# ethz-asl/object_keypoints

Measured on AMD Instinct MI355X. Metric: frames/sec keypoint inference (511x511 -> heatmaps+3D), higher is better.
Workload: dtype bf16; 1 GPU; BASELINE configs[2]: batch=64/GPU synthetic 511x511 frames, bf16 activations+weights, fp32 accumulate, CornerNet-Squeeze K=3 (valve) random-init procedural weights; fp32 NCHW frames -> stem -> hourglass+heads; peak-NMS -> depth lifting -> object grouping on injected bump scenes (SURVEY 8(d), 1-2 objects/frame); frames_per_gpu=64, global_batch=64, parallelism=frame-dp1, resident_frame_batches=4

## Files before the change

object_keypoints_amd/csrc/okp_fire2.hip:

```cpp
#include <cstdio>
#include <cstring>

#include <cstdlib>

#include "okp_internal.h"

#ifdef OKP_F2_ABL_NOSTORE
#define F2_STORE_(v, rs, off) do { if ((off) == 0x7ffffff0u) __builtin_amdgcn_raw_buffer_store_b128(v, rs, (int)(off), 0, 0); } while (0)
#else
#define F2_STORE_(v, rs, off) __builtin_amdgcn_raw_buffer_store_b128(v, rs, (int)(off), 0, 0)
#endif
#define F2_STORE(v, rs, off) do { \
    if constexpr (G) { if ((uint32_t)(off) < kInvalid) range_h = okp_range_max_h8(range_h, v); } \
    F2_STORE_(v, rs, off); } while (0)


namespace {

constexpr uint32_t kInvalid = 0x80000000u;
typedef __attribute__((address_space(3))) void* lds_ptr_t;
typedef float f32x2 __attribute__((ext_vector_type(2)));

constexpr int SP = 128;
constexpr int PBI = 6;
// ... 50 lines not shown
    case 5: asm volatile("s_waitcnt vmcnt(5)" ::: "memory"); break;
    case 6: asm volatile("s_waitcnt vmcnt(6)" ::: "memory"); break;
    case 7: asm volatile("s_waitcnt vmcnt(7)" ::: "memory"); break;
    default: asm volatile("s_waitcnt vmcnt(8)" ::: "memory"); break;
  }
}

#ifdef OKP_FIRE_STAMPS
#define F2_STAMP_ANY(i) do { if (lane == 0 && blockIdx.x < 16) { uint64_t t_; asm volatile("s_memtime %0\n s_waitcnt lgkmcnt(0)" : "=s"(t_) :: "memory"); p.dbg[(blockIdx.x * 8 + w) * 8 + (i)] = (uint32_t)t_; } } while (0)
#define F2_STAMP(i) do { if (second && lane == 0 && blockIdx.x < 16) { uint64_t t_; asm volatile("s_memtime %0\n s_waitcnt lgkmcnt(0)" : "=s"(t_) :: "memory"); p.dbg[(blockIdx.x * 8 + w) * 8 + (i)] = (uint32_t)t_; } } while (0)
#else
#define F2_STAMP(i) do {} while (0)
#define F2_STAMP_ANY(i) do {} while (0)
#endif

template <typename T, int CIN, int MID, int STR, bool DWM = false, bool G = false>
__global__ __launch_bounds__(MID * 2, MID == 128 ? 2 : 1) void okp_fire2_kernel(const OkpFire2Params p) {
  static_assert(STR == 1 || STR == 2, "stride of both branches");
  static_assert(!G || std::is_same<T, _Float16>::value, "the 16-bit storage guard is an fp16 instantiation");
  constexpr bool DWM2 = DWM && STR == 2;
  constexpr int D2H = 3, D2W = 8, D2SW = 2 * (D2W - 1) + 3, D2SH = 2 * (D2H - 1) + 3, D2B = 2;
  static_assert(D2SH * D2SW <= SP && D2B * 16 >= D2H * D2W + 8, "stride-2 matrix-pipe tile");
  constexpr int DIH = kDwmIH;
  constexpr int DSW = 18;
  constexpr int NSB = !DWM ? SP / 16 : STR == 1 ? ((DIH + 2) * DSW + 15) / 16 : (D2SH * D2SW + 15) / 16;
  constexpr int NW = MID / 32;
  constexpr int NT = 64 * NW;
  constexpr int HALF = MID;
  constexpr int KS1 = CIN / 32;
  constexpr int KS2 = MID / 32;
#ifdef OKP_F2_RESIDENT_W1
  constexpr bool RES = CIN <= 256;
  constexpr int DWB = 1;
#else
  constexpr bool RES = false;
#ifdef OKP_F2_RESIDENT_WA
  constexpr int DWB = (CIN == 256 && MID == 128) ? OKP_F2_RESIDENT_WA : 1;
#else
  constexpr int DWB = (CIN == 256 && MID == 128) ? 4 : 1;
#endif
// ... 94 lines not shown
    const int row = 16 * (w + NW * i) + (lane >> 2);
    d_sy[i] = fastdiv(row, p.div_sw);
    d_sx[i] = row - d_sy[i] * p.SW;
    if (row >= p.SH * p.SW) d_sy[i] = 1 << 20;
    d_chunk[i] = (uint32_t)(((lane & 3) - 2 * (row >> 2)) & 3) * 16u;
  }
  const int m_sy = tid < p.SH * p.SW ? fastdiv(tid, p.div_sw) : (1 << 20);
  const int m_sx = tid - fastdiv(tid, p.div_sw) * p.SW;

  auto tile_origin = [&](int slot, int& n, int& y0, int& x0) {
    const int xq = p.n_tiles >> 3, xr = p.n_tiles & 7, xcd = slot & 7;
    const int tile = (xcd < xr ? xcd * (xq + 1) : xr * (xq + 1) + (xcd - xr) * xq) + (slot >> 3);
    n = fastdiv(tile, p.div_tiles_frame);
    const int trem = tile - n * p.tiles_y * p.tiles_x;
    const int ty = fastdiv(trem, p.div_tiles_x);
    y0 = ty * p.IH;
    x0 = (trem - ty * p.tiles_x) * p.IW;
  };
  uint32_t d_off[NDM];
  auto tile_setup = [&](int tile) {
    int n, y0, x0;
    tile_origin(tile, n, y0, x0);
#pragma unroll
    for (int i = 0; i < NDM; ++i) {
      const int y = STR * y0 - 1 + d_sy[i], x = STR * x0 - 1 + d_sx[i];
      const bool ok = y >= 0 && y < p.H && x >= 0 && x < p.W;
      d_off[i] = ok ? (uint32_t)(((long)n * p.H + y) * p.W + x) * (uint32_t)(p.x_ps * 2) + d_chunk[i] : kInvalid;
    }
    if (tid < SP) {
      const int y = STR * y0 - 1 + m_sy, x = STR * x0 - 1 + m_sx;
      const unsigned long long m = __ballot(y >= 0 && y < p.H && x >= 0 && x < p.W);
      if (lane == 0) {
        uint32_t* mk = reinterpret_cast<uint32_t*>(smem + OFF_MASK);
        mk[2 * w] = (uint32_t)m;
        mk[2 * w + 1] = (uint32_t)(m >> 32);
      }
    }
  };
#ifdef OKP_F2_ABL_NOX
  bool abl_started = false;
#endif
  auto issue_x = [&](int ks, int stage) {
#ifdef OKP_F2_ABL_NOX
    if (abl_started) return;
#endif
#pragma unroll
    for (int i = 0; i < NDM; ++i)
      if (UNI || i < nd)
        __builtin_amdgcn_raw_ptr_buffer_load_lds(rs_x, (lds_ptr_t)(smem + OFF_X + stage * XST + (w + NW * i) * 1024), 16,
                                                 (int)(d_off[i] == kInvalid ? kInvalid : d_off[i] + (uint32_t)ks * 64u), 0, 0, 0);
  };

  int tile = blockIdx.x;
  if (tile >= p.n_tiles) return;
  F2_STAMP_ANY(5);
  tile_setup(tile);
  first_weights(w1f);
#pragma unroll
  for (int ks = 0; ks < NST - 1; ++ks) issue_x(ks, ks);
  {
    static_assert(10 * HALF == 5 * NT, "depth-wise constants per thread");
    float cv[5];
#pragma unroll
    for (int k = 0; k < 5; ++k) {
      const int i = tid + k * NT;
      cv[k] = *(i < 9 * HALF ? p.wd + i : p.bd + (i - 9 * HALF));
    }
#pragma unroll
    for (int k = 0; k < 5; ++k) {
      const int i = tid + k * NT;
      if constexpr (DWM) {
        const uint32_t wq = (i & 1) ? okp_pack2<T>(0.f, cv[k]) : okp_pack2<T>(cv[k], 0.f);
        reinterpret_cast<uint32_t*>(smem + OFF_WD)[i] = i < 9 * HALF ? wq : __builtin_bit_cast(uint32_t, cv[k]);
      } else {
        reinterpret_cast<float*>(smem + OFF_WD)[i] = cv[k];
      }
    }
  }
  if (tid < 16 * PBI) {
    const int iy = fastdiv(tid, p.div_iw), ix = tid - iy * p.IW;
    reinterpret_cast<uint32_t*>(smem + OFF_TAB)[tid] = tid < p.IP ? (uint32_t)(iy * p.W + ix) * (uint32_t)(p.x_ps * 2) : kInvalid;
    reinterpret_cast<uint32_t*>(smem + OFF_TAB)[96 + tid] = tid < p.IP ? (uint32_t)(iy * p.Wo + ix) * (uint32_t)(p.out_ps * 2) : kInvalid;
  }

  __syncthreads();
  F2_STAMP_ANY(6);

  uint32_t range_h = 0u;
  for (; tile < p.n_tiles; tile += gridDim.x) {
    int n, y0, x0;
    tile_origin(tile, n, y0, x0);
#ifdef OKP_FIRE_STAMPS
    const bool second = tile == (int)(blockIdx.x + gridDim.x);
#endif
    F2_STAMP(0);
    int qt = q, tidt = tid;
    asm volatile("" : "+v"(qt), "+v"(tidt));
#ifdef OKP_F2_NO_REMAP
    const int dw_cg = tidt % CG, dw_slot = tidt / CG;
#else
    const int dw_l = tidt & 31;
    const int dw_cg = CG == 16 ? ((dw_l & 3) | ((dw_l >> 1) & 12)) : tidt % CG;
    const int dw_slot = CG == 16 ? 4 * (tidt >> 6) + 2 * ((tidt >> 5) & 1) + (((dw_l >> 2) ^ (dw_l >> 3) ^ (dw_l >> 4)) & 1) : tidt / CG;
#endif
    auto load_col_residuals = [&](int ix, u32x4 (&rr)[MAXIH], uint32_t (&oo)[MAXIH]) {
      const int cg = dw_cg;
      const int ox = x0 + ix;
      const uint32_t pix = (uint32_t)(((long)n * p.Ho + y0) * p.Wo + ox);
// ... 9 lines not shown
            const int row = (iy + 1) * p.SW + (ix < p.IW ? ix : 0) + 1;
            rr[iy] = *reinterpret_cast<const u32x4*>(smem + OFF_X + ((KS1 / 2 + (cg >> 2)) % NST) * XST + row * 64 + (((cg & 3) + 2 * (row >> 2)) & 3) * 16);
          } else {
            rr[iy] = __builtin_amdgcn_raw_buffer_load_b128(rs_x, (int)(ok ? xo : kInvalid), 0, 0);
          }
        }
        xo += (uint32_t)(p.W * p.x_ps * 2);
        oof += (uint32_t)(p.Wo * p.out_ps * 2);
      }
    };
    uint32_t o_off[PBI];
    u32x4 r_raw[PBI];
    u32x4 rr[MAXIH];
    uint32_t oo[MAXIH];

    f32x4 acc[NSB][2];
#pragma unroll
    for (int pb = 0; pb < NSB; ++pb) {
      acc[pb][0] = b1v0;
      acc[pb][1] = b1v1;
    }
    if constexpr (PIPE) {
      u32x4 a[2][NSB];
#pragma unroll
      for (int ks = 0; ks <= KS1; ++ks) {
        if (ks < KS1) {
          if (ks == 0) wait_vm(0);
          else if (ks >= 3) wait_vm(2 + (ks + 1 < KS1 ? nd + 2 : 0) + (ks + 2 < KS1 ? nd : 0));
          asm volatile("s_waitcnt lgkmcnt(0)" ::: "memory");
          __builtin_amdgcn_s_barrier();
          if (ks + 2 < KS1) load_w1(ks + 2, w1f[(ks + 2) % NWS]);
          if (ks + NST - 1 < KS1) issue_x(ks + NST - 1, (ks + NST - 1) % NST);
          const char* st = smem + OFF_X + (ks % NST) * XST + xfrag_off;
#pragma unroll
          for (int pb = 0; pb < NSB; ++pb) a[ks & 1][pb] = *reinterpret_cast<const u32x4*>(st + pb * 1024);
          __builtin_amdgcn_sched_barrier(0);
        }
        if (ks > 0) {
#pragma unroll
          for (int pb = 0; pb < NSB; ++pb)
#pragma unroll
            for (int b = 0; b < 2; ++b)
              acc[pb][b] = H16<T>::mfma16(w1f[(ks - 1) % NWS][b], a[(ks - 1) & 1][pb], acc[pb][b]);
          __builtin_amdgcn_sched_barrier(0);
        }
      }
    } else
#pragma unroll
    for (int ks = 0; ks < KS1; ++ks) {
      if (ks == 0) wait_vm(0);
      else if constexpr (WRING) {
        auto nw = [](int j) { return j >= 1 && j - 1 + DW < KS1 ? 2 : 0; };
        auto nx = [](int j) { return j >= 0 && j + NST - 1 < KS1 ? 1 : 0; };
        wait_vm((DW >= 4 ? nw(ks - 2) : 0) + nw(ks - 1) + (nx(ks - 2) + nx(ks - 1)) * nd);
      } else if (ks >= (RES ? NST - 1 : 2))
        wait_vm((ks + 1 < KS1 ? nd + (RES ? 0 : 2) : 0) + (ks + 2 < KS1 ? nd : 0));
      asm volatile("s_waitcnt lgkmcnt(0)" ::: "memory");
      __builtin_amdgcn_s_barrier();
      if constexpr (WRING) { if (ks >= 1 && ks - 1 + DW < KS1) issue_w(ks - 1 + DW); }
      else if constexpr (!RES) { if (ks + 2 < KS1) load_w1(ks + 2, w1f[(ks + 2) % 3]); }
      if (ks + NST - 1 < KS1) issue_x(ks + NST - 1, (ks + NST - 1) % NST);
      const char* st = smem + OFF_X + (ks % NST) * XST + xfrag_off;
      u32x4 a[NSB], wr[2] = {};
      if constexpr (WRING) {
#pragma unroll
        for (int b = 0; b < 2; ++b) wr[b] = *reinterpret_cast<const u32x4*>(smem + OFF_W1 + ((ks % DW) * NW + w) * 2048 + b * 1024 + lane * 16);
      }
#pragma unroll
      for (int pb = 0; pb < NSB; ++pb) a[pb] = *reinterpret_cast<const u32x4*>(st + pb * 1024);
#ifdef OKP_F2_PIN_READS
      __builtin_amdgcn_sched_barrier(0);
#endif
#pragma unroll
      for (int pb = 0; pb < NSB; ++pb)
#pragma unroll
        for (int b = 0; b < 2; ++b)
          acc[pb][b] = H16<T>::mfma16(WRING ? wr[b] : w1f[RES ? ks : ks % 3][b], a[pb], acc[pb][b]);
    }
    F2_STAMP(1);
#ifdef OKP_F2_ABL_NOX
    abl_started = true;
#endif
    if constexpr (!RESWA) {
#pragma unroll
      for (int b = 0; b < 2; ++b)
#pragma unroll
        for (int ks = 0; ks < KS2; ++ks) {
#ifdef OKP_F2_ABL_NOWEIGHTS
          if (b + ks != 0) { waf[b][ks] = u32x4{0x3c003c00u, 0u, 0u, 0u}; continue; }
#endif
          waf[b][ks] = wa_lane[(size_t)(b * KS2 + ks) * 64];
        }
    }
    {
      const uint32_t* mk = reinterpret_cast<const uint32_t*>(smem + OFF_MASK);
      int l16t = l16;
      asm volatile("" : "+v"(l16t));
      uint32_t mq[4];
#pragma unroll
      for (int i = 0; i < 4; ++i) mq[i] = mk[i] >> l16t;
#pragma unroll
      for (int pb = 0; pb < NSB; ++pb) {
        const bool ok = (mq[pb >> 1] >> (16 * (pb & 1))) & 1u;
        u32x4 v;
#pragma unroll
        for (int b = 0; b < 2; ++b) {
          const uint32_t p0 = okp_pack2<T>(acc[pb][b][0], acc[pb][b][1]), p1 = okp_pack2<T>(acc[pb][b][2], acc[pb][b][3]);
          v[2 * b] = ok ? p0 : 0u;
          v[2 * b + 1] = ok ? p1 : 0u;
        }
        if constexpr (G) range_h = okp_range_max_h8(range_h, v);
        *reinterpret_cast<u32x4*>(smem + s_dst + pb * 16 * (MID * 2)) = v;
      }
    }
    __syncthreads();
    F2_STAMP(2);
    uint32_t dwm_o[DIH];
    uint32_t d2_o[D2B];
    if constexpr (DWM2) {
      int l16t = l16;
      asm volatile("" : "+v"(l16t));
      const int liy = l16t >> 3, lix = l16t & 7;
      const uint32_t pix0 = (uint32_t)(((long)n * p.Ho + y0) * p.Wo + x0);
      const uint32_t lane_o = (uint32_t)(liy * p.Wo + lix) * (uint32_t)(p.out_ps * 2) + (uint32_t)chq * 2u;
      const bool col_ok = lix < p.IW && x0 + lix < p.Wo;
      f32x4 ac2[D2B][2];
#pragma unroll
      for (int pb = 0; pb < D2B; ++pb) {
        const int iy = 2 * pb + liy;
        const bool ok = col_ok && iy < p.IH && y0 + iy < p.Ho;
        d2_o[pb] = ok ? lane_o + (pix0 + (uint32_t)(2 * pb * p.Wo)) * (uint32_t)(p.out_ps * 2) : kInvalid;
// ... 18 lines not shown
#pragma unroll
      for (int pb = 0; pb < D2B; ++pb) {
        const u32x4 v = relu_add_pack8<T>(ac2[pb][0], ac2[pb][1], u32x4{0u, 0u, 0u, 0u});
        F2_STORE(v, rs_o, d2_o[pb]);
      }
    } else if constexpr (DWM) {
      int l16t = l16;
      asm volatile("" : "+v"(l16t));
      const uint32_t pix0 = (uint32_t)(((long)n * p.Ho + y0) * p.Wo + x0);
      const uint32_t lane_x = (uint32_t)l16t * (uint32_t)(p.x_ps * 2) + (uint32_t)chq * 2u, lane_o = (uint32_t)l16t * (uint32_t)(p.out_ps * 2) + (uint32_t)chq * 2u;
      u32x4 rsk[DIH];
      const uint32_t rowx = (uint32_t)(p.W * p.x_ps * 2), rowo = (uint32_t)(p.Wo * p.out_ps * 2), noskip = p.skip ? 0u : kInvalid;
      uint32_t sx = pix0 * (uint32_t)(p.x_ps * 2), so = pix0 * (uint32_t)(p.out_ps * 2);
#pragma unroll
      for (int iy = 0; iy < DIH; ++iy) {
        const uint32_t bad = (iy < p.IH && y0 + iy < p.Ho) ? 0u : kInvalid;
        dwm_o[iy] = lane_o + (so | bad);
        rsk[iy] = __builtin_amdgcn_raw_buffer_load_b128(rs_x, (int)(lane_x + (sx | bad | noskip)), 0, 0);
        sx += rowx;
        so += rowo;
      }
      f32x4 ac2[DIH][2];
#pragma unroll
      for (int iy = 0; iy < DIH; ++iy) {
        ac2[iy][0] = bav0;
        ac2[iy][1] = bav1;
      }
      const uint32_t s_lane = (uint32_t)OFF_S + (uint32_t)(DSW + 1 + l16t) * (uint32_t)(MID * 2);
#pragma unroll
      for (int ks = 0; ks < KS2; ++ks) {
        u32x4 a[DIH];
#pragma unroll
        for (int iy = 0; iy < DIH; ++iy) {
          const uint32_t key = (uint32_t)(l16t + (iy + 1) * DSW + 1) & (uint32_t)SWM;
          a[iy] = *reinterpret_cast<const u32x4*>(smem + s_lane + (uint32_t)(iy * DSW * MID * 2) + (((uint32_t)(4 * ks + qt) ^ key) << 4));
        }
#pragma unroll
        for (int iy = 0; iy < DIH; ++iy)
#pragma unroll
          for (int b = 0; b < 2; ++b)
            ac2[iy][b] = H16<T>::mfma16(waf[b][ks], a[iy], ac2[iy][b]);
      }
#pragma unroll
      for (int iy = 0; iy < DIH; ++iy) {
        const u32x4 v = relu_add_pack8<T>(ac2[iy][0], ac2[iy][1], rsk[iy]);
        F2_STORE(v, rs_o, dwm_o[iy]);
      }
    } else {
      const bool full = y0 + p.IH <= p.Ho && x0 + p.IW <= p.Wo;
      const uint32_t pix0 = (uint32_t)(((long)n * p.Ho + y0) * p.Wo + x0);
// ... 38 lines not shown
      for (int pb = 0; pb < PBI; ++pb) {
        if (16 * pb < p.IP) {
          const u32x4 v = relu_add_pack8<T>(ac2[pb][0], ac2[pb][1], r_raw[pb]);
          F2_STORE(v, rs_o, o_off[pb]);
        }
      }
    }
    asm volatile("" ::: "memory");
    F2_STAMP(3);

    if constexpr (DWM2) {
      int l16t = l16;
      asm volatile("" : "+v"(l16t));
      const int liy = l16t >> 3, lix = l16t & 7;
      {
        const int next = tile + gridDim.x;
        if (next < p.n_tiles) {
          tile_setup(next);
          first_weights(w1f);
#pragma unroll
          for (int ks = 0; ks < NST - 1; ++ks) issue_x(ks, ks);
        }
      }
      const float* const bl = reinterpret_cast<const float*>(smem + OFF_WD) + 9 * HALF + chq;
      const f32x4 bdv0 = *reinterpret_cast<const f32x4*>(bl), bdv1 = *reinterpret_cast<const f32x4*>(bl + 4);
      f32x4 acd[D2B][2];
#pragma unroll
      for (int pb = 0; pb < D2B; ++pb) { acd[pb][0] = bdv0; acd[pb][1] = bdv1; }
      const uint32_t am = (qt == (l16t >> 2)) ? 0xffffffffu : 0u;
      const uint32_t m_lo = (l16t & 2) ? 0u : am, m_hi = (l16t & 2) ? am : 0u;
      const uint32_t wt_lane = (uint32_t)OFF_WD + (uint32_t)(chq + (l16t & 3)) * 4u;
      const uint32_t cx = (uint32_t)(4 * w) + (uint32_t)qt;
      const uint32_t sp_lane = (uint32_t)(2 * liy * D2SW + 2 * lix);
      u32x4 a0 = {0u, 0u, 0u, 0u}, a1 = {0u, 0u, 0u, 0u};
#pragma unroll
      for (int tap = 0; tap < 9; ++tap) {
        const int dy = tap / 3, dx = tap % 3;
// ... 17 lines not shown
      for (int pb = 0; pb < D2B; ++pb) {
        const u32x4 o = relu_add_pack8<T>(acd[pb][0], acd[pb][1], u32x4{0u, 0u, 0u, 0u});
        F2_STORE(o, rs_o, d2_o[pb] == kInvalid ? kInvalid : d2_o[pb] + (uint32_t)(HALF * 2));
      }
    } else if constexpr (DWM) {
      int l16t = l16;
      asm volatile("" : "+v"(l16t));
      u32x4 rr2[DIH];
      uint32_t oo2[DIH];
#pragma unroll
      for (int iy = 0; iy < DIH; ++iy) {
        oo2[iy] = dwm_o[iy] + (uint32_t)(HALF * 2);
        rr2[iy] = u32x4{0u, 0u, 0u, 0u};
        if (p.skip) {
          if constexpr (RING_SKIP) {
            const uint32_t row = (uint32_t)((iy + 1) * DSW + 1) + (uint32_t)l16t;
            rr2[iy] = *reinterpret_cast<const u32x4*>(smem + OFF_X + ((KS1 / 2 + w) % NST) * XST + row * 64u + (((uint32_t)qt + 2u * (row >> 2)) & 3u) * 16u);
          } else {
            const bool ok = iy < p.IH && y0 + iy < p.Ho;
            const uint32_t pix0 = (uint32_t)(((long)n * p.Ho + y0) * p.Wo + x0);
            const uint32_t sx = ok ? (pix0 + (uint32_t)(iy * p.W)) * (uint32_t)(p.x_ps * 2) : kInvalid;
            rr2[iy] = __builtin_amdgcn_raw_buffer_load_b128(rs_x, (int)((uint32_t)l16t * (uint32_t)(p.x_ps * 2) + (uint32_t)(HALF + chq) * 2u + sx), 0, 0);
          }
        }
      }
      if constexpr (RING_SKIP) {
        if (p.skip) { asm volatile("s_waitcnt lgkmcnt(0)" ::: "memory"); __syncthreads(); }
      }
      {
        const int next = tile + gridDim.x;
        if (next < p.n_tiles) {
          tile_setup(next);
          first_weights(w1f);
#pragma unroll
          for (int ks = 0; ks < NST - 1; ++ks) issue_x(ks, ks);
        }
      }
      const float* const bl = reinterpret_cast<const float*>(smem + OFF_WD) + 9 * HALF + chq;
      const f32x4 bdv0 = *reinterpret_cast<const f32x4*>(bl), bdv1 = *reinterpret_cast<const f32x4*>(bl + 4);
      f32x4 acd[DIH][2];
#pragma unroll
      for (int iy = 0; iy < DIH; ++iy) { acd[iy][0] = bdv0; acd[iy][1] = bdv1; }
      const uint32_t am = (qt == (l16t >> 2)) ? 0xffffffffu : 0u;
      const uint32_t m_lo = (l16t & 2) ? 0u : am, m_hi = (l16t & 2) ? am : 0u;
      const uint32_t wt_lane = (uint32_t)OFF_WD + (uint32_t)(chq + (l16t & 3)) * 4u;
      const uint32_t cx = (uint32_t)(4 * w) + (uint32_t)qt;
#ifndef OKP_F2_ABL_NODW
      u32x4 a0[3], a1[3];
#pragma unroll
      for (int dy = 0; dy < 3; ++dy) { a0[dy] = u32x4{0u, 0u, 0u, 0u}; a1[dy] = u32x4{0u, 0u, 0u, 0u}; }
#pragma unroll
      for (int dx = 0; dx < 3; ++dx) {
#pragma unroll
        for (int dy = 0; dy < 3; ++dy) {
          const uint32_t v0 = *reinterpret_cast<const uint32_t*>(smem + wt_lane + ((dy * 3 + dx) * HALF) * 4);
          const uint32_t v1 = *reinterpret_cast<const uint32_t*>(smem + wt_lane + ((dy * 3 + dx) * HALF + 4) * 4);
          a0[dy][0] = v0 & m_lo; a0[dy][1] = v0 & m_hi;
          a1[dy][2] = v1 & m_lo; a1[dy][3] = v1 & m_hi;
        }
        u32x4 bf[DIH + 2];
#pragma unroll
        for (int r = 0; r < DIH + 2; ++r) {
          const uint32_t sp = (uint32_t)(r * DSW + dx) + (uint32_t)l16t;
          bf[r] = *reinterpret_cast<const u32x4*>(smem + OFF_S + sp * (MID * 2) + ((cx ^ (sp & SWM)) << 4));
        }
#pragma unroll
        for (int r = 0; r < DIH + 2; ++r) {
#pragma unroll
          for (int dy = 0; dy < 3; ++dy) {
            const int iy = r - dy;
            if (iy >= 0 && iy < DIH) {
              acd[iy][0] = H16<T>::mfma16(a0[dy], bf[r], acd[iy][0]);
              acd[iy][1] = H16<T>::mfma16(a1[dy], bf[r], acd[iy][1]);
            }
          }
        }
      }
#endif
// ... 8 lines not shown
      const float* const wl = reinterpret_cast<const float*>(smem + OFF_WD) + cg * 8;
      float breg[8];
      {
        const f32x4 u0 = *reinterpret_cast<const f32x4*>(wl + 9 * HALF), u1 = *reinterpret_cast<const f32x4*>(wl + 9 * HALF + 4);
#pragma unroll
        for (int e = 0; e < 4; ++e) { breg[e] = u0[e]; breg[4 + e] = u1[e]; }
      }
      bool prefetched = false;
      for (int ix = dw_slot; ix < ((p.IW + 15) & ~15); ix += 16) {
        load_col_residuals(ix, rr, oo);
        if (RING_SKIP ? ix + 16 >= ((p.IW + 15) & ~15) : !prefetched) {
          prefetched = true;
          if constexpr (RING_SKIP) {
            if (p.skip) { asm volatile("s_waitcnt lgkmcnt(0)" ::: "memory"); __syncthreads(); }
          }
          const int next = tile + gridDim.x;
          if (next < p.n_tiles) {
            tile_setup(next);
            first_weights(w1f);
#pragma unroll
            for (int ks = 0; ks < NST - 1; ++ks) issue_x(ks, ks);
          }
        }
        const int ixc = ix < p.IW ? ix : 0;
        f32x2 v[MAXIH][4];
#pragma unroll
        for (int iy = 0; iy < MAXIH; ++iy)
#pragma unroll
          for (int e = 0; e < 4; ++e) v[iy][e] = f32x2{breg[2 * e], breg[2 * e + 1]};
#pragma unroll
        for (int dx = 0; dx < 3; ++dx) {
          f32x2 wt[3][4];
#pragma unroll
          for (int dy = 0; dy < 3; ++dy) {
            const f32x4 u0 = *reinterpret_cast<const f32x4*>(wl + (dy * 3 + dx) * HALF), u1 = *reinterpret_cast<const f32x4*>(wl + (dy * 3 + dx) * HALF + 4);
            wt[dy][0] = f32x2{u0[0], u0[1]}; wt[dy][1] = f32x2{u0[2], u0[3]}; wt[dy][2] = f32x2{u1[0], u1[1]}; wt[dy][3] = f32x2{u1[2], u1[3]};
          }
// ... 52 lines not shown
        }
#pragma unroll
        for (int iy = 0; iy < MAXIH; ++iy) {
          u32x4 o;
#pragma unroll
          for (int e = 0; e < 4; ++e) {
            const float lo = fmaxf(v[iy][e][0] + H16<T>::lo(rr[iy][e]), 0.f);
            const float hi = fmaxf(v[iy][e][1] + H16<T>::hi(rr[iy][e]), 0.f);
            o[e] = okp_pack2<T>(lo, hi);
          }
          F2_STORE(o, rs_o, oo[iy]);
        }
      }
    }
    F2_STAMP(4);
  }
  if constexpr (G) okp_raise_range_flag(p.range_flag, okp_range_exceeded_h2(range_h));
  F2_STAMP_ANY(7);
}

}


bool okp_fire2_supported(int cin, int mid, int half, int stride) {
  if (half != mid) return false;
  if (stride == 1)
    return (cin == 256 && mid == 128) || (cin == 384 && mid == 192) || (cin == 512 && mid == 256) ||
           (cin == 384 && mid == 128) || (cin == 512 && mid == 192);
  return stride == 2 && ((cin == 256 && mid == 128) || (cin == 384 && mid == 192) || (cin == 384 && mid == 256) || (cin == 256 && mid == 192));
}
// ... 13 lines not shown
    }
  if (stride == 2) {
    static const char* const e = getenv("OKP_F2_S2_TILE");
    int ih = 0, iw = 0;
    if (e && sscanf(e, "%d,%d", &ih, &iw) == 2 && ih >= 1 && ih <= MAXIH && iw >= 1 && (2 * (ih - 1) + 3) * (2 * (iw - 1) + 3) <= SP && ih * iw <= 16 * PBI) {
      p.IH = ih < p.Ho ? ih : p.Ho; p.IW = iw < p.Wo ? iw : p.Wo; p.SH = 2 * (p.IH - 1) + 3; p.SW = 2 * (p.IW - 1) + 3;
      p.tiles_y = (p.Ho + p.IH - 1) / p.IH; p.tiles_x = (p.Wo + p.IW - 1) / p.IW;
    }
  }
  static const bool dwm_on = [] { const char* e = getenv("OKP_F2_DWM"); return !(e && e[0] == '0'); }();
  static const int dwm_mid = [] { const char* e = getenv("OKP_F2_DWM_MID"); return e ? atoi(e) : 256; }();
  const bool dwm = dwm_on && stride == 1 && p.Wo % 16 == 0 && mid <= dwm_mid;
  if (dwm) {
    p.IH = p.Ho < kDwmIH ? p.Ho : kDwmIH; p.IW = 16; p.SH = p.IH + 2; p.SW = 18;
    p.tiles_y = (p.Ho + p.IH - 1) / p.IH; p.tiles_x = p.Wo / 16;
  }
  static const bool dwm2_on = [] { const char* e = getenv("OKP_F2_DWM_S2"); return !(e && e[0] == '0'); }();
  const bool dwm2 = dwm_on && dwm2_on && stride == 2 && p.Wo % 8 == 0 && mid <= dwm_mid;
  if (dwm2) {
    const long tx = p.Wo / 8;
    int ih = p.Ho < 3 ? p.Ho : 3;
    if (ih == 3 && (long)p.N * ((p.Ho + 1) / 2) * tx <= resident_wg) ih = 2;
    p.IH = ih; p.IW = 8; p.SH = 2 * (ih - 1) + 3; p.SW = 17;
    p.tiles_y = (p.Ho + ih - 1) / ih; p.tiles_x = (int)tx;
  }
  p.IP = p.IH * p.IW;
  p.RPR = (p.IW + 3) / 4;
  const long tiles = (long)p.N * p.tiles_y * p.tiles_x;
  if (tiles >= 0x7FFFFFFFl) { okp_set_error("okp_fire_forward: too many tiles"); return OKP_EINVAL; }
  p.n_tiles = (int)tiles;
// ... 21 lines not shown
      for (int w = 0; w < nw; ++w) {
        const uint32_t* a = &h[(wg * 8 + w) * 8];
        if (!a[4]) continue;
        if (wg % 5 == 0 && (w == 0 || w == nw - 1)) printf("wg %2d wave %d: %6u | %6u | %6u | %6u\n", wg, w, a[1] - a[0], a[2] - a[1], a[3] - a[2], a[4] - a[3]);
        for (int i = 0; i < 4; ++i) sum[i] += a[i + 1] - a[i];
        ++cnt;
      }
    if (cnt) printf("mean: %.0f | %.0f | %.0f | %.0f  = %.0f clocks per tile\n", sum[0] / cnt, sum[1] / cnt, sum[2] / cnt, sum[3] / cnt, (sum[0] + sum[1] + sum[2] + sum[3]) / cnt);
    double pro = 0, all = 0; int c2 = 0;
    for (int wg = 0; wg < 16; ++wg)
      for (int w = 0; w < nw; ++w) { const uint32_t* a = &h[(wg * 8 + w) * 8]; if (!a[7]) continue; pro += a[6] - a[5]; all += a[7] - a[5]; ++c2; }
    if (c2) printf("whole kernel: prologue (first requests + constants -> LDS + barrier) %.0f clocks, entry to exit %.0f clocks\n", pro / c2, all / c2);
  } } print_at_exit{p, mid, stream, dbg};
#endif
  bool launched = true;
  if (stride == 1 && dwm) {
    if (cin == 256 && mid == 128) hipLaunchKernelGGL((okp_fire2_kernel<T, 256, 128, 1, true, G>), grid, block, 0, stream, p);
    else if (cin == 384 && mid == 192) hipLaunchKernelGGL((okp_fire2_kernel<T, 384, 192, 1, true, G>), grid, block, 0, stream, p);
    else if (cin == 512 && mid == 256) hipLaunchKernelGGL((okp_fire2_kernel<T, 512, 256, 1, true, G>), grid, block, 0, stream, p);
    else if (cin == 384 && mid == 128) hipLaunchKernelGGL((okp_fire2_kernel<T, 384, 128, 1, true, G>), grid, block, 0, stream, p);
    else if (cin == 512 && mid == 192) hipLaunchKernelGGL((okp_fire2_kernel<T, 512, 192, 1, true, G>), grid, block, 0, stream, p);
    else launched = false;
  } else if (stride == 2 && dwm2) {
    if (cin == 256 && mid == 128) hipLaunchKernelGGL((okp_fire2_kernel<T, 256, 128, 2, true, G>), grid, block, 0, stream, p);
    else if (cin == 384 && mid == 192) hipLaunchKernelGGL((okp_fire2_kernel<T, 384, 192, 2, true, G>), grid, block, 0, stream, p);
    else if (cin == 384 && mid == 256) hipLaunchKernelGGL((okp_fire2_kernel<T, 384, 256, 2, true, G>), grid, block, 0, stream, p);
    else if (cin == 256 && mid == 192) hipLaunchKernelGGL((okp_fire2_kernel<T, 256, 192, 2, true, G>), grid, block, 0, stream, p);
    else launched = false;
  } else if constexpr (G) {
    okp_set_error("okp_fire_forward: the range-guarded fp16 one-launch kernel takes output maps %d wide at stride %d only on its matrix-pipe form "
                  "(width a multiple of %d); run the squeeze plan and the fused tail", p.Wo, stride, stride == 1 ? 16 : 8);
    return OKP_EINVAL;
  } else if (stride == 1) {
    if (cin == 256 && mid == 128) hipLaunchKernelGGL((okp_fire2_kernel<T, 256, 128, 1>), grid, block, 0, stream, p);
    else if (cin == 384 && mid == 192) hipLaunchKernelGGL((okp_fire2_kernel<T, 384, 192, 1>), grid, block, 0, stream, p);
    else if (cin == 512 && mid == 256) hipLaunchKernelGGL((okp_fire2_kernel<T, 512, 256, 1>), grid, block, 0, stream, p);
    else if (cin == 384 && mid == 128) hipLaunchKernelGGL((okp_fire2_kernel<T, 384, 128, 1>), grid, block, 0, stream, p);
    else if (cin == 512 && mid == 192) hipLaunchKernelGGL((okp_fire2_kernel<T, 512, 192, 1>), grid, block, 0, stream, p);
    else launched = false;
  } else {
    if (cin == 256 && mid == 192) hipLaunchKernelGGL((okp_fire2_kernel<T, 256, 192, 2>), grid, block, 0, stream, p);
    else if (cin == 256 && mid == 128) hipLaunchKernelGGL((okp_fire2_kernel<T, 256, 128, 2>), grid, block, 0, stream, p);
// ... 74 lines not shown
```

object_keypoints_amd/csrc/okp_internal.h:

```cpp
#pragma once
#include <hip/hip_runtime.h>
#include <stdint.h>
#include "okp.h"

#define OKP_MAX_TAPS 32

typedef float f32x4 __attribute__((ext_vector_type(4)));
typedef float f32x16 __attribute__((ext_vector_type(16)));
typedef __bf16 bf16x8 __attribute__((ext_vector_type(8)));
typedef __bf16 bf16x4 __attribute__((ext_vector_type(4)));
typedef __bf16 bf16x2 __attribute__((ext_vector_type(2)));
typedef _Float16 f16x8 __attribute__((ext_vector_type(8)));
typedef _Float16 f16x4 __attribute__((ext_vector_type(4)));
typedef _Float16 f16x2 __attribute__((ext_vector_type(2)));
typedef unsigned int u32x4 __attribute__((ext_vector_type(4)));
typedef unsigned int u32x2 __attribute__((ext_vector_type(2)));

template <typename T> struct H16;
template <> struct H16<__bf16> {
  using x2 = bf16x2; using x4 = bf16x4; using x8 = bf16x8;
  static constexpr int kDtype = OKP_BF16;
  static __device__ __forceinline__ f32x4 mfma16(const u32x4& a, const u32x4& b, const f32x4& c) {
#if defined(__HIP_DEVICE_COMPILE__)
    return __builtin_amdgcn_mfma_f32_16x16x32_bf16(__builtin_bit_cast(bf16x8, a), __builtin_bit_cast(bf16x8, b), c, 0, 0, 0);
// ... 189 lines not shown
#ifdef OKP_PATCH_STAMPS
  uint32_t* dbg;
#endif
};

struct OkpFire2Params {
  const void* x; uint32_t x_bytes; int32_t H, W, x_ps;
  void* out; uint32_t out_bytes; int32_t Ho, Wo, out_ps;
  int32_t N, skip;
  const void* w1; int32_t w1_cout_pad; const float* b1;
  const void* wa; int32_t wa_cout_pad; const float* ba;
  const float* wd; const float* bd;
  const float* s1; const float* sa;
  int32_t* range_flag;
  int32_t SH, SW, IH, IW, IP, RPR, tiles_y, tiles_x, n_tiles;
  OkpFastDiv div_tiles_frame, div_tiles_x, div_sw, div_iw, div_rpr;
#ifdef OKP_FIRE_STAMPS
  uint32_t* dbg;
#endif
};

struct OkpFireChainModule {
  const void* w1; int32_t w1_cout_pad; const float* b1;
  const void* wa; int32_t wa_cout_pad; const float* ba;
  const float* wd; const float* bd;
};
struct OkpFireChainParams {
  const void* x; void* out; int32_t x_ps, out_ps, H, W, n_modules;
  int32_t He, We;
  OkpFireChainModule mod[OKP_FIRE_CHAIN_MAX];
// ... 99 lines not shown
```

Before: 12820 frames/s.

## Walk vertical strips in fire2 kernel reusing squeeze halo rows via ring buffer

Adds a STRIP variant of the stride-1 matrix-pipe fire kernel. Each workgroup walks a vertical segment of output rows tile by tile and keeps the squeezed activations in a ring buffer in LDS, so successive tiles recompute only the new rows instead of the two halo rows each time. The host chooses the segment height with a simple cost model, or takes it from environment variables. This cuts redundant squeeze GEMM work and input loads, at the price of fewer independent tiles (less parallelism) and more complex indexing and skip handling.

```diff
diff --git a/object_keypoints_amd/csrc/okp_fire2.hip b/object_keypoints_amd/csrc/okp_fire2.hip
--- a/object_keypoints_amd/csrc/okp_fire2.hip
+++ b/object_keypoints_amd/csrc/okp_fire2.hip
@@ -2,6 +2,7 @@
 #include <cstring>
 
 #include <cstdlib>
+#include <type_traits>
 
 #include "okp_internal.h"
 
@@ -88,9 +89,10 @@
 #define F2_STAMP_ANY(i) do {} while (0)
 #endif
 
-template <typename T, int CIN, int MID, int STR, bool DWM = false, bool G = false>
+template <typename T, int CIN, int MID, int STR, bool DWM = false, bool STRIP = false, bool G = false>
 __global__ __launch_bounds__(MID * 2, MID == 128 ? 2 : 1) void okp_fire2_kernel(const OkpFire2Params p) {
   static_assert(STR == 1 || STR == 2, "stride of both branches");
+  static_assert(!STRIP || (DWM && STR == 1), "the strip walk is a form of the stride-1 matrix-pipe instances");
   static_assert(!G || std::is_same<T, _Float16>::value, "the 16-bit storage guard is an fp16 instantiation");
   constexpr bool DWM2 = DWM && STR == 2;
   constexpr int D2H = 3, D2W = 8, D2SW = 2 * (D2W - 1) + 3, D2SH = 2 * (D2H - 1) + 3, D2B = 2;
@@ -98,6 +100,8 @@
   constexpr int DIH = kDwmIH;
   constexpr int DSW = 18;
   constexpr int NSB = !DWM ? SP / 16 : STR == 1 ? ((DIH + 2) * DSW + 15) / 16 : (D2SH * D2SW + 15) / 16;
+  constexpr int RP = (DIH + 2) * DSW;
+  constexpr int NBF = (RP + 15) / 16, NBN = (DIH * DSW + 15) / 16;
   constexpr int NW = MID / 32;
   constexpr int NT = 64 * NW;
   constexpr int HALF = MID;
@@ -222,22 +226,21 @@
     n = fastdiv(tile, p.div_tiles_frame);
     const int trem = tile - n * p.tiles_y * p.tiles_x;
     const int ty = fastdiv(trem, p.div_tiles_x);
-    y0 = ty * p.IH;
+    y0 = ty * (STRIP ? p.seg_rows : p.IH);
     x0 = (trem - ty * p.tiles_x) * p.IW;
   };
   uint32_t d_off[NDM];
-  auto tile_setup = [&](int tile) {
-    int n, y0, x0;
-    tile_origin(tile, n, y0, x0);
+  auto tile_setup = [&](int n, int y0, int x0, bool first) {
+    const int yt = STRIP && !first ? y0 + 1 : STR * y0 - 1, rows = STRIP && !first ? DIH : 1 << 20;
 #pragma unroll
     for (int i = 0; i < NDM; ++i) {
-      const int y = STR * y0 - 1 + d_sy[i], x = STR * x0 - 1 + d_sx[i];
-      const bool ok = y >= 0 && y < p.H && x >= 0 && x < p.W;
+      const int y = yt + d_sy[i], x = STR * x0 - 1 + d_sx[i];
+      const bool ok = y >= 0 && y < p.H && x >= 0 && x < p.W && (!STRIP || d_sy[i] < rows);
       d_off[i] = ok ? (uint32_t)(((long)n * p.H + y) * p.W + x) * (uint32_t)(p.x_ps * 2) + d_chunk[i] : kInvalid;
     }
     if (tid < SP) {
-      const int y = STR * y0 - 1 + m_sy, x = STR * x0 - 1 + m_sx;
-      const unsigned long long m = __ballot(y >= 0 && y < p.H && x >= 0 && x < p.W);
+      const int y = yt + m_sy, x = STR * x0 - 1 + m_sx;
+      const unsigned long long m = __ballot(y >= 0 && y < p.H && x >= 0 && x < p.W && (!STRIP || m_sy < rows));
       if (lane == 0) {
         uint32_t* mk = reinterpret_cast<uint32_t*>(smem + OFF_MASK);
         mk[2 * w] = (uint32_t)m;
@@ -248,24 +251,40 @@
 #ifdef OKP_F2_ABL_NOX
   bool abl_started = false;
 #endif
-  auto issue_x = [&](int ks, int stage) {
+  auto issue_x = [&](int ks, int stage, int nb) {
 #ifdef OKP_F2_ABL_NOX
     if (abl_started) return;
 #endif
 #pragma unroll
     for (int i = 0; i < NDM; ++i)
-      if (UNI || i < nd)
+      if (STRIP ? (NW * (i + 1) <= nb || w + NW * i < nb) : (UNI || i < nd))
         __builtin_amdgcn_raw_ptr_buffer_load_lds(rs_x, (lds_ptr_t)(smem + OFF_X + stage * XST + (w + NW * i) * 1024), 16,
                                                  (int)(d_off[i] == kInvalid ? kInvalid : d_off[i] + (uint32_t)ks * 64u), 0, 0, 0);
   };
 
   int tile = blockIdx.x;
   if (tile >= p.n_tiles) return;
+  int n, y0, x0, ye = 0;
+  bool first = true;
+  uint32_t rs = 0;
+  tile_origin(tile, n, y0, x0);
+  if constexpr (STRIP) ye = min(y0 + p.seg_rows, p.Ho);
+  auto next_tile = [&](int& t2, int& n2, int& y2, int& x2, int& ye2, bool& first2) -> bool {
+    if constexpr (STRIP) {
+      if (y0 + DIH < ye) { t2 = tile; n2 = n; y2 = y0 + DIH; x2 = x0; ye2 = ye; first2 = false; return true; }
+    }
+    t2 = tile + gridDim.x;
+    if (t2 >= p.n_tiles) return false;
+    tile_origin(t2, n2, y2, x2);
+    first2 = true;
+    if constexpr (STRIP) ye2 = min(y2 + p.seg_rows, p.Ho);
+    return true;
+  };
   F2_STAMP_ANY(5);
-  tile_setup(tile);
+  tile_setup(n, y0, x0, true);
   first_weights(w1f);
 #pragma unroll
-  for (int ks = 0; ks < NST - 1; ++ks) issue_x(ks, ks);
+  for (int ks = 0; ks < NST - 1; ++ks) issue_x(ks, ks, NBF);
   {
     static_assert(10 * HALF == 5 * NT, "depth-wise constants per thread");
     float cv[5];
@@ -295,11 +314,24 @@
   F2_STAMP_ANY(6);
 
   uint32_t range_h = 0u;
-  for (; tile < p.n_tiles; tile += gridDim.x) {
-    int n, y0, x0;
-    tile_origin(tile, n, y0, x0);
 #ifdef OKP_FIRE_STAMPS
-    const bool second = tile == (int)(blockIdx.x + gridDim.x);
+  int tile_no = 0;
+#endif
+  auto prefetch_next = [&]() {
+    int tile2 = 0, n2 = 0, y2 = 0, x2 = 0, ye2 = 0;
+    bool first2 = true;
+    if (next_tile(tile2, n2, y2, x2, ye2, first2)) {
+      tile_setup(n2, y2, x2, first2);
+      first_weights(w1f);
+#pragma unroll
+      for (int ks = 0; ks < NST - 1; ++ks) {
+        if (STRIP && !first2) issue_x(ks, ks, NBN); else issue_x(ks, ks, NBF);
+      }
+    }
+  };
+  for (;;) {
+#ifdef OKP_FIRE_STAMPS
+    const bool second = STRIP ? ++tile_no == 2 : tile == (int)(blockIdx.x + gridDim.x);
 #endif
     F2_STAMP(0);
     int qt = q, tidt = tid;
@@ -339,31 +371,39 @@
     u32x4 rr[MAXIH];
     uint32_t oo[MAXIH];
 
-    f32x4 acc[NSB][2];
-#pragma unroll
-    for (int pb = 0; pb < NSB; ++pb) {
+    auto squeeze_phase = [&](auto first_c) {
+    constexpr bool FIRST = decltype(first_c)::value;
+    constexpr int NB = !STRIP ? NSB : FIRST ? NBF : NBN;
+    constexpr int JL = FIRST ? RP : DIH * DSW;
+    const int ndt = !STRIP ? nd : NB % NW == 0 ? NB / NW : w < NB ? (NB - w + NW - 1) / NW : 0;
+    uint32_t wbase = FIRST ? 0u : rs + (uint32_t)(2 * DSW);
+    wbase = wbase >= (uint32_t)RP ? wbase - (uint32_t)RP : wbase;
+    (void)JL; (void)wbase;
+    f32x4 acc[NB][2];
+#pragma unroll
+    for (int pb = 0; pb < NB; ++pb) {
       acc[pb][0] = b1v0;
       acc[pb][1] = b1v1;
     }
     if constexpr (PIPE) {
-      u32x4 a[2][NSB];
+      u32x4 a[2][NB];
 #pragma unroll
       for (int ks = 0; ks <= KS1; ++ks) {
         if (ks < KS1) {
           if (ks == 0) wait_vm(0);
-          else if (ks >= 3) wait_vm(2 + (ks + 1 < KS1 ? nd + 2 : 0) + (ks + 2 < KS1 ? nd : 0));
+          else if (ks >= 3) wait_vm(2 + (ks + 1 < KS1 ? ndt + 2 : 0) + (ks + 2 < KS1 ? ndt : 0));
           asm volatile("s_waitcnt lgkmcnt(0)" ::: "memory");
           __builtin_amdgcn_s_barrier();
           if (ks + 2 < KS1) load_w1(ks + 2, w1f[(ks + 2) % NWS]);
-          if (ks + NST - 1 < KS1) issue_x(ks + NST - 1, (ks + NST - 1) % NST);
+          if (ks + NST - 1 < KS1) issue_x(ks + NST - 1, (ks + NST - 1) % NST, NB);
           const char* st = smem + OFF_X + (ks % NST) * XST + xfrag_off;
 #pragma unroll
-          for (int pb = 0; pb < NSB; ++pb) a[ks & 1][pb] = *reinterpret_cast<const u32x4*>(st + pb * 1024);
+          for (int pb = 0; pb < NB; ++pb) a[ks & 1][pb] = *reinterpret_cast<const u32x4*>(st + pb * 1024);
           __builtin_amdgcn_sched_barrier(0);
         }
         if (ks > 0) {
 #pragma unroll
-          for (int pb = 0; pb < NSB; ++pb)
+          for (int pb = 0; pb < NB; ++pb)
 #pragma unroll
             for (int b = 0; b < 2; ++b)
               acc[pb][b] = H16<T>::mfma16(w1f[(ks - 1) % NWS][b], a[(ks - 1) & 1][pb], acc[pb][b]);
@@ -377,27 +417,27 @@
       else if constexpr (WRING) {
         auto nw = [](int j) { return j >= 1 && j - 1 + DW < KS1 ? 2 : 0; };
         auto nx = [](int j) { return j >= 0 && j + NST - 1 < KS1 ? 1 : 0; };
-        wait_vm((DW >= 4 ? nw(ks - 2) : 0) + nw(ks - 1) + (nx(ks - 2) + nx(ks - 1)) * nd);
+        wait_vm((DW >= 4 ? nw(ks - 2) : 0) + nw(ks - 1) + (nx(ks - 2) + nx(ks - 1)) * ndt);
       } else if (ks >= (RES ? NST - 1 : 2))
-        wait_vm((ks + 1 < KS1 ? nd + (RES ? 0 : 2) : 0) + (ks + 2 < KS1 ? nd : 0));
+        wait_vm((ks + 1 < KS1 ? ndt + (RES ? 0 : 2) : 0) + (ks + 2 < KS1 ? ndt : 0));
       asm volatile("s_waitcnt lgkmcnt(0)" ::: "memory");
       __builtin_amdgcn_s_barrier();
       if constexpr (WRING) { if (ks >= 1 && ks - 1 + DW < KS1) issue_w(ks - 1 + DW); }
       else if constexpr (!RES) { if (ks + 2 < KS1) load_w1(ks + 2, w1f[(ks + 2) % 3]); }
-      if (ks + NST - 1 < KS1) issue_x(ks + NST - 1, (ks + NST - 1) % NST);
+      if (ks + NST - 1 < KS1) issue_x(ks + NST - 1, (ks + NST - 1) % NST, NB);
       const char* st = smem + OFF_X + (ks % NST) * XST + xfrag_off;
-      u32x4 a[NSB], wr[2] = {};
+      u32x4 a[NB], wr[2] = {};
       if constexpr (WRING) {
 #pragma unroll
         for (int b = 0; b < 2; ++b) wr[b] = *reinterpret_cast<const u32x4*>(smem + OFF_W1 + ((ks % DW) * NW + w) * 2048 + b * 1024 + lane * 16);
       }
 #pragma unroll
-      for (int pb = 0; pb < NSB; ++pb) a[pb] = *reinterpret_cast<const u32x4*>(st + pb * 1024);
+      for (int pb = 0; pb < NB; ++pb) a[pb] = *reinterpret_cast<const u32x4*>(st + pb * 1024);
 #ifdef OKP_F2_PIN_READS
       __builtin_amdgcn_sched_barrier(0);
 #endif
 #pragma unroll
-      for (int pb = 0; pb < NSB; ++pb)
+      for (int pb = 0; pb < NB; ++pb)
 #pragma unroll
         for (int b = 0; b < 2; ++b)
           acc[pb][b] = H16<T>::mfma16(WRING ? wr[b] : w1f[RES ? ks : ks % 3][b], a[pb], acc[pb][b]);
@@ -425,7 +465,7 @@
 #pragma unroll
       for (int i = 0; i < 4; ++i) mq[i] = mk[i] >> l16t;
 #pragma unroll
-      for (int pb = 0; pb < NSB; ++pb) {
+      for (int pb = 0; pb < NB; ++pb) {
         const bool ok = (mq[pb >> 1] >> (16 * (pb & 1))) & 1u;
         u32x4 v;
 #pragma unroll
@@ -435,11 +475,27 @@
           v[2 * b + 1] = ok ? p1 : 0u;
         }
         if constexpr (G) range_h = okp_range_max_h8(range_h, v);
+        if constexpr (STRIP) {
+          uint32_t t = wbase + (uint32_t)(16 * pb) + (uint32_t)l16t;
+          t = t >= (uint32_t)RP ? t - (uint32_t)RP : t;
+          if (16 * pb + 15 < JL || l16t < JL - 16 * pb)
+            *reinterpret_cast<u32x4*>(smem + OFF_S + t * (uint32_t)(MID * 2) + ((((uint32_t)(4 * w) + (uint32_t)qt) ^ (t & (uint32_t)SWM)) << 4)) = v;
+        } else
         *reinterpret_cast<u32x4*>(smem + s_dst + pb * 16 * (MID * 2)) = v;
       }
+    }
+    };
+    if constexpr (STRIP) {
+      if (first) squeeze_phase(std::true_type{}); else squeeze_phase(std::false_type{});
+    } else {
+      squeeze_phase(std::true_type{});
     }
     __syncthreads();
     F2_STAMP(2);
+    auto rowpix = [&](int r) -> uint32_t {
+      if constexpr (STRIP) { const uint32_t t = rs + (uint32_t)(r * DSW); return t >= (uint32_t)RP ? t - (uint32_t)RP : t; }
+      return (uint32_t)(r * DSW);
+    };
     uint32_t dwm_o[DIH];
     uint32_t d2_o[D2B];
     if constexpr (DWM2) {
@@ -488,7 +544,7 @@
       uint32_t sx = pix0 * (uint32_t)(p.x_ps * 2), so = pix0 * (uint32_t)(p.out_ps * 2);
 #pragma unroll
       for (int iy = 0; iy < DIH; ++iy) {
-        const uint32_t bad = (iy < p.IH && y0 + iy < p.Ho) ? 0u : kInvalid;
+        const uint32_t bad = (STRIP ? y0 + iy < ye : (iy < p.IH && y0 + iy < p.Ho)) ? 0u : kInvalid;
         dwm_o[iy] = lane_o + (so | bad);
         rsk[iy] = __builtin_amdgcn_raw_buffer_load_b128(rs_x, (int)(lane_x + (sx | bad | noskip)), 0, 0);
         sx += rowx;
@@ -500,14 +556,13 @@
         ac2[iy][0] = bav0;
         ac2[iy][1] = bav1;
       }
-      const uint32_t s_lane = (uint32_t)OFF_S + (uint32_t)(DSW + 1 + l16t) * (uint32_t)(MID * 2);
 #pragma unroll
       for (int ks = 0; ks < KS2; ++ks) {
         u32x4 a[DIH];
 #pragma unroll
         for (int iy = 0; iy < DIH; ++iy) {
-          const uint32_t key = (uint32_t)(l16t + (iy + 1) * DSW + 1) & (uint32_t)SWM;
-          a[iy] = *reinterpret_cast<const u32x4*>(smem + s_lane + (uint32_t)(iy * DSW * MID * 2) + (((uint32_t)(4 * ks + qt) ^ key) << 4));
+          const uint32_t sp = rowpix(iy + 1) + 1u + (uint32_t)l16t;
+          a[iy] = *reinterpret_cast<const u32x4*>(smem + OFF_S + sp * (uint32_t)(MID * 2) + (((uint32_t)(4 * ks + qt) ^ (sp & (uint32_t)SWM)) << 4));
         }
 #pragma unroll
         for (int iy = 0; iy < DIH; ++iy)
@@ -576,13 +631,7 @@
       asm volatile("" : "+v"(l16t));
       const int liy = l16t >> 3, lix = l16t & 7;
       {
-        const int next = tile + gridDim.x;
-        if (next < p.n_tiles) {
-          tile_setup(next);
-          first_weights(w1f);
-#pragma unroll
-          for (int ks = 0; ks < NST - 1; ++ks) issue_x(ks, ks);
-        }
+        prefetch_next();
       }
       const float* const bl = reinterpret_cast<const float*>(smem + OFF_WD) + 9 * HALF + chq;
       const f32x4 bdv0 = *reinterpret_cast<const f32x4*>(bl), bdv1 = *reinterpret_cast<const f32x4*>(bl + 4);
@@ -630,10 +679,16 @@
         rr2[iy] = u32x4{0u, 0u, 0u, 0u};
         if (p.skip) {
           if constexpr (RING_SKIP) {
-            const uint32_t row = (uint32_t)((iy + 1) * DSW + 1) + (uint32_t)l16t;
+            const bool in_ring = !STRIP || first || iy > 0;
+            const uint32_t row = (uint32_t)((STRIP && !first && iy > 0 ? iy - 1 : iy + 1) * DSW + 1) + (uint32_t)l16t;
             rr2[iy] = *reinterpret_cast<const u32x4*>(smem + OFF_X + ((KS1 / 2 + w) % NST) * XST + row * 64u + (((uint32_t)qt + 2u * (row >> 2)) & 3u) * 16u);
+            if (STRIP && iy == 0) {
+              const uint32_t sx = in_ring ? kInvalid : (uint32_t)(((long)n * p.Ho + y0) * p.Wo + x0) * (uint32_t)(p.x_ps * 2);
+              const u32x4 g = __builtin_amdgcn_raw_buffer_load_b128(rs_x, (int)((uint32_t)l16t * (uint32_t)(p.x_ps * 2) + (uint32_t)(HALF + chq) * 2u + sx), 0, 0);
+              rr2[iy] = in_ring ? rr2[iy] : g;
+            }
           } else {
-            const bool ok = iy < p.IH && y0 + iy < p.Ho;
+            const bool ok = STRIP ? y0 + iy < ye : (iy < p.IH && y0 + iy < p.Ho);
             const uint32_t pix0 = (uint32_t)(((long)n * p.Ho + y0) * p.Wo + x0);
             const uint32_t sx = ok ? (pix0 + (uint32_t)(iy * p.W)) * (uint32_t)(p.x_ps * 2) : kInvalid;
             rr2[iy] = __builtin_amdgcn_raw_buffer_load_b128(rs_x, (int)((uint32_t)l16t * (uint32_t)(p.x_ps * 2) + (uint32_t)(HALF + chq) * 2u + sx), 0, 0);
@@ -644,13 +699,7 @@
         if (p.skip) { asm volatile("s_waitcnt lgkmcnt(0)" ::: "memory"); __syncthreads(); }
       }
       {
-        const int next = tile + gridDim.x;
-        if (next < p.n_tiles) {
-          tile_setup(next);
-          first_weights(w1f);
-#pragma unroll
-          for (int ks = 0; ks < NST - 1; ++ks) issue_x(ks, ks);
-        }
+        prefetch_next();
       }
       const float* const bl = reinterpret_cast<const float*>(smem + OFF_WD) + 9 * HALF + chq;
       const f32x4 bdv0 = *reinterpret_cast<const f32x4*>(bl), bdv1 = *reinterpret_cast<const f32x4*>(bl + 4);
@@ -677,7 +726,7 @@
         u32x4 bf[DIH + 2];
 #pragma unroll
         for (int r = 0; r < DIH + 2; ++r) {
-          const uint32_t sp = (uint32_t)(r * DSW + dx) + (uint32_t)l16t;
+          const uint32_t sp = rowpix(r) + (uint32_t)dx + (uint32_t)l16t;
           bf[r] = *reinterpret_cast<const u32x4*>(smem + OFF_S + sp * (MID * 2) + ((cx ^ (sp & SWM)) << 4));
         }
 #pragma unroll
@@ -716,13 +765,7 @@
           if constexpr (RING_SKIP) {
             if (p.skip) { asm volatile("s_waitcnt lgkmcnt(0)" ::: "memory"); __syncthreads(); }
           }
-          const int next = tile + gridDim.x;
-          if (next < p.n_tiles) {
-            tile_setup(next);
-            first_weights(w1f);
-#pragma unroll
-            for (int ks = 0; ks < NST - 1; ++ks) issue_x(ks, ks);
-          }
+          prefetch_next();
         }
         const int ixc = ix < p.IW ? ix : 0;
         f32x2 v[MAXIH][4];
@@ -805,6 +848,11 @@
       }
     }
     F2_STAMP(4);
+    if (!next_tile(tile, n, y0, x0, ye, first)) break;
+    if constexpr (STRIP) {
+      rs = first ? 0u : rs + (uint32_t)(DIH * DSW);
+      rs = rs >= (uint32_t)RP ? rs - (uint32_t)RP : rs;
+    }
   }
   if constexpr (G) okp_raise_range_flag(p.range_flag, okp_range_exceeded_h2(range_h));
   F2_STAMP_ANY(7);
@@ -848,6 +896,27 @@
   if (dwm) {
     p.IH = p.Ho < kDwmIH ? p.Ho : kDwmIH; p.IW = 16; p.SH = p.IH + 2; p.SW = 18;
     p.tiles_y = (p.Ho + p.IH - 1) / p.IH; p.tiles_x = p.Wo / 16;
+  }
+  bool strip = false;
+  if (dwm && mid <= 192) {
+    const char* e = getenv("OKP_F2_STRIP");
+    const char* es = getenv("OKP_F2_SEG_ROWS");
+    const int forced = es ? atoi(es) : 0;
+    if (!(e && e[0] == '0')) {
+      constexpr long kFixed = 87, kBlock = 10, kNbf = ((kDwmIH + 2) * 18 + 15) / 16, kNbn = (kDwmIH * 18 + 15) / 16;
+      const long tx = p.Wo / 16;
+      long best_cost = (((long)p.N * p.tiles_y * tx + resident_wg - 1) / resident_wg) * (kFixed + kBlock * kNbf);
+      for (int s = kDwmIH + 1; s <= p.Ho; ++s) {
+        const long segs = (long)p.N * ((p.Ho + s - 1) / s) * tx, t = (s + kDwmIH - 1) / kDwmIH;
+        const long cost = ((segs + resident_wg - 1) / resident_wg) * (t * kFixed + kBlock * (kNbf + (t - 1) * kNbn));
+        if (cost < best_cost) { best_cost = cost; p.seg_rows = s; strip = true; }
+      }
+      if (forced >= 1) { p.seg_rows = forced < p.Ho ? forced : p.Ho; strip = true; }
+    }
+    if (strip) {
+      p.IH = kDwmIH; p.SH = kDwmIH + 2;
+      p.tiles_y = (p.Ho + p.seg_rows - 1) / p.seg_rows;
+    }
   }
   static const bool dwm2_on = [] { const char* e = getenv("OKP_F2_DWM_S2"); return !(e && e[0] == '0'); }();
   const bool dwm2 = dwm_on && dwm2_on && stride == 2 && p.Wo % 8 == 0 && mid <= dwm_mid;
@@ -899,18 +968,24 @@
   } } print_at_exit{p, mid, stream, dbg};
 #endif
   bool launched = true;
-  if (stride == 1 && dwm) {
-    if (cin == 256 && mid == 128) hipLaunchKernelGGL((okp_fire2_kernel<T, 256, 128, 1, true, G>), grid, block, 0, stream, p);
-    else if (cin == 384 && mid == 192) hipLaunchKernelGGL((okp_fire2_kernel<T, 384, 192, 1, true, G>), grid, block, 0, stream, p);
-    else if (cin == 512 && mid == 256) hipLaunchKernelGGL((okp_fire2_kernel<T, 512, 256, 1, true, G>), grid, block, 0, stream, p);
-    else if (cin == 384 && mid == 128) hipLaunchKernelGGL((okp_fire2_kernel<T, 384, 128, 1, true, G>), grid, block, 0, stream, p);
-    else if (cin == 512 && mid == 192) hipLaunchKernelGGL((okp_fire2_kernel<T, 512, 192, 1, true, G>), grid, block, 0, stream, p);
+  if (stride == 1 && dwm && strip) {
+    if (cin == 256 && mid == 128) hipLaunchKernelGGL((okp_fire2_kernel<T, 256, 128, 1, true, true, G>), grid, block, 0, stream, p);
+    else if (cin == 384 && mid == 192) hipLaunchKernelGGL((okp_fire2_kernel<T, 384, 192, 1, true, true, G>), grid, block, 0, stream, p);
+    else if (cin == 384 && mid == 128) hipLaunchKernelGGL((okp_fire2_kernel<T, 384, 128, 1, true, true, G>), grid, block, 0, stream, p);
+    else if (cin == 512 && mid == 192) hipLaunchKernelGGL((okp_fire2_kernel<T, 512, 192, 1, true, true, G>), grid, block, 0, stream, p);
+    else launched = false;
+  } else if (stride == 1 && dwm) {
+    if (cin == 256 && mid == 128) hipLaunchKernelGGL((okp_fire2_kernel<T, 256, 128, 1, true, false, G>), grid, block, 0, stream, p);
+    else if (cin == 384 && mid == 192) hipLaunchKernelGGL((okp_fire2_kernel<T, 384, 192, 1, true, false, G>), grid, block, 0, stream, p);
+    else if (cin == 512 && mid == 256) hipLaunchKernelGGL((okp_fire2_kernel<T, 512, 256, 1, true, false, G>), grid, block, 0, stream, p);
+    else if (cin == 384 && mid == 128) hipLaunchKernelGGL((okp_fire2_kernel<T, 384, 128, 1, true, false, G>), grid, block, 0, stream, p);
+    else if (cin == 512 && mid == 192) hipLaunchKernelGGL((okp_fire2_kernel<T, 512, 192, 1, true, false, G>), grid, block, 0, stream, p);
     else launched = false;
   } else if (stride == 2 && dwm2) {
-    if (cin == 256 && mid == 128) hipLaunchKernelGGL((okp_fire2_kernel<T, 256, 128, 2, true, G>), grid, block, 0, stream, p);
-    else if (cin == 384 && mid == 192) hipLaunchKernelGGL((okp_fire2_kernel<T, 384, 192, 2, true, G>), grid, block, 0, stream, p);
-    else if (cin == 384 && mid == 256) hipLaunchKernelGGL((okp_fire2_kernel<T, 384, 256, 2, true, G>), grid, block, 0, stream, p);
-    else if (cin == 256 && mid == 192) hipLaunchKernelGGL((okp_fire2_kernel<T, 256, 192, 2, true, G>), grid, block, 0, stream, p);
+    if (cin == 256 && mid == 128) hipLaunchKernelGGL((okp_fire2_kernel<T, 256, 128, 2, true, false, G>), grid, block, 0, stream, p);
+    else if (cin == 384 && mid == 192) hipLaunchKernelGGL((okp_fire2_kernel<T, 384, 192, 2, true, false, G>), grid, block, 0, stream, p);
+    else if (cin == 384 && mid == 256) hipLaunchKernelGGL((okp_fire2_kernel<T, 384, 256, 2, true, false, G>), grid, block, 0, stream, p);
+    else if (cin == 256 && mid == 192) hipLaunchKernelGGL((okp_fire2_kernel<T, 256, 192, 2, true, false, G>), grid, block, 0, stream, p);
     else launched = false;
   } else if constexpr (G) {
     okp_set_error("okp_fire_forward: the range-guarded fp16 one-launch kernel takes output maps %d wide at stride %d only on its matrix-pipe form "
diff --git a/object_keypoints_amd/csrc/okp_internal.h b/object_keypoints_amd/csrc/okp_internal.h
--- a/object_keypoints_amd/csrc/okp_internal.h
+++ b/object_keypoints_amd/csrc/okp_internal.h
@@ -227,6 +227,7 @@
   const float* s1; const float* sa;
   int32_t* range_flag;
   int32_t SH, SW, IH, IW, IP, RPR, tiles_y, tiles_x, n_tiles;
+  int32_t seg_rows;
   OkpFastDiv div_tiles_frame, div_tiles_x, div_sw, div_iw, div_rpr;
 #ifdef OKP_FIRE_STAMPS
   uint32_t* dbg;
```

Result: slower. 12570 frames/s (-1.9%).
